# OpenVVC/VVCSoftware_VTM

Hardware: AMD Instinct MI355X
Metric: encoded frames/sec (bit-exact bitstream) at 4K10 RA QP32, 1/2/4/8 GPU [M1: hot-path pictures/s of the kernels behind the call sites, NOT EncoderApp fps] (higher is better)
Workload: dtype int16

## Files before the change

vvcsoftware_vtm_amd/csrc/interp.hip:

```cpp
#include "common.h"
#include "dist_dev.h"
#include "mfma_tr.h"

static_assert(offsetof(vvcgpu_mc_desc, dst_stride) == 32 && offsetof(vvcgpu_mc_desc, w) == 36 && offsetof(vvcgpu_mc_desc, frac_x0) == 40 &&
              offsetof(vvcgpu_mc_desc, is_luma) == 44 && sizeof(vvcgpu_mc_desc) == 48, "vvcgpu_mc_desc layout");

namespace {

__constant__ short c_lumaFilter[16][8] = {
  {  0, 0,   0, 64,  0,   0,  0,  0 }, {  0, 1,  -3, 63,  4,  -2,  1,  0 }, { -1, 2,  -5, 62,  8,  -3,  1,  0 },
  { -1, 3,  -8, 60, 13,  -4,  1,  0 }, { -1, 4, -10, 58, 17,  -5,  1,  0 }, { -1, 4, -11, 52, 26,  -8,  3, -1 },
  { -1, 3,  -9, 47, 31, -10,  4, -1 }, { -1, 4, -11, 45, 34, -10,  4, -1 }, { -1, 4, -11, 40, 40, -11,  4, -1 },
  { -1, 4, -10, 34, 45, -11,  4, -1 }, { -1, 4, -10, 31, 47,  -9,  3, -1 }, { -1, 3,  -8, 26, 52, -11,  4, -1 },
  {  0, 1,  -5, 17, 58, -10,  4, -1 }, {  0, 1,  -4, 13, 60,  -8,  3, -1 }, {  0, 1,  -3,  8, 62,  -5,  2, -1 },
  {  0, 1,  -2,  4, 63,  -3,  1,  0 } };
__constant__ short c_chromaFilter[32][4] = {
  {  0, 64,  0,  0 }, { -1, 63,  2,  0 }, { -2, 62,  4,  0 }, { -2, 60,  7, -1 }, { -2, 58, 10, -2 }, { -3, 57, 12, -2 },
  { -4, 56, 14, -2 }, { -4, 55, 15, -2 }, { -4, 54, 16, -2 }, { -5, 53, 18, -2 }, { -6, 52, 20, -2 }, { -6, 49, 24, -3 },
  { -6, 46, 28, -4 }, { -5, 44, 29, -4 }, { -4, 42, 30, -4 }, { -4, 39, 33, -4 }, { -4, 36, 36, -4 }, { -4, 33, 39, -4 },
  { -4, 30, 42, -4 }, { -4, 29, 44, -5 }, { -4, 28, 46, -6 }, { -3, 24, 49, -6 }, { -2, 20, 52, -6 }, { -2, 18, 53, -5 },
  { -2, 16, 54, -4 }, { -2, 15, 55, -4 }, { -2, 14, 56, -4 }, { -2, 12, 57, -3 }, { -2, 10, 58, -2 }, { -1,  7, 60, -2 },
  {  0,  4, 62, -2 }, {  0,  2, 63, -1 } };

constexpr int IF_INTERNAL_PREC = 14, IF_FILTER_PREC = 6, IF_INTERNAL_OFFS = 1 << 13;
// ... 697 lines not shown
  {
    const int ix = (int)(short)(raw.flg >> 16);
    const vvcgpu_wp_param eA = wp_load(wp, __builtin_amdgcn_readlane(ix, 0)), eB = wp_load(wp, __builtin_amdgcn_readlane(ix, 8));
    o = mm_tail_wp(K, fr[0], fr[1], bi == 1, K.c16 >= 8 ? eB : eA);
  }
  else o = mm_tail(K, fr[0], fr[1], bi == 1 ? 1.f : 0.f, bi == 1 ? K.scBi2 : 1.f, bi == 1 ? K.ofBi2 : 1024.f, bi == 0 && (fx0 | fy0) == 0);
  const bool outB = K.c16 >= 8;
  if ((K.g >> 1) == (K.c16 >> 3) && (outB ? (hasB && !badB) : !badA))
  {
    const long long dstOff = (long long)(((unsigned long long)raw.dstHi << 32) | raw.dstLo);
    Pel* dp = dstBase + dstOff + (ptrdiff_t)(K.c16 & 7) * (int)raw.ds + 4 * (K.g & 1);
    reinterpret_cast<MmQuad*>(dp)->v = o;
  }
}

__device__ __forceinline__ int mm_kind_of(const uint4& q)
{
  vvcgpu_mc_desc d;
  d.w = (short)(q.y & 0xFFFFu); d.h = (short)(q.y >> 16);
  d.frac_x0 = (signed char)(q.z & 0xFFu); d.frac_y0 = (signed char)((q.z >> 8) & 0xFFu); d.frac_x1 = (signed char)((q.z >> 16) & 0xFFu); d.frac_y1 = (signed char)(q.z >> 24);
  d.is_luma = (signed char)(q.w & 0xFFu); d.bi = (signed char)((q.w >> 8) & 0xFFu);
  return mm_kind(d);
}
struct MmServe { const Pel* ref0Base; const Pel* ref1Base; Pel* dstBase; const vvcgpu_mc_desc* descs; const int* flags; int n, bd, cmin, cmax, w0, W, luma; };
struct MmServeWp : MmServe { const vvcgpu_wp_param* wp; int nWp, allGen; };
template <bool WPF> __device__ __forceinline__ void mm_second_pass(const MmServe* sv, short* gen, unsigned* genT);
__device__ __noinline__ void mm_serve_one(const MmServe* sv, int li, short* gen, unsigned* genT);
__device__ __noinline__ void mm_serve_one_wp(const MmServeWp* sv, int li, short* gen, unsigned* genT);
constexpr int MM_SKIP = 3;
__device__ __forceinline__ int mm_wp_kind(int k, const uint4& q2, const vvcgpu_wp_param* __restrict__ wp, int nWp, int bd, int allGen)
{
  if (wp_skip(q2, wp, nWp, bd)) return MM_SKIP;
  return allGen && k > 0 ? 0 : k;
}
constexpr int MM_GEN_SHORTS = 23 * 24 + 23 * 16;

template <int KIND_T>
__global__ __launch_bounds__(256, 4) void mc_mfma_kernel(const Pel* __restrict__ ref0Base, const Pel* __restrict__ ref1Base, Pel* __restrict__ dstBase,
                                                                         const vvcgpu_mc_desc* __restrict__ descs, int n, int bd, int cmin, int cmax,
                                                                         const _Float16* __restrict__ image, int* __restrict__ flags, unsigned long long* __restrict__ diag,
                                                                         int* __restrict__ genCount, int* __restrict__ nextCounters, int serve)
{
  constexpr bool WPF = false;
  const vvcgpu_wp_param* const wp = nullptr;
  const int nWp = 0, allGen = 0;
#include "mc_mfma_body.inc"
}
// ... 203 lines not shown
  static_assert(MM_GEN_SHORTS == WR * WP + WR * ST, "LDS of the generic body inside mc_mfma_kernel");
  const MmServe S = *sv;
  const vvcgpu_mc_desc d = S.descs[li];
  mc_generic_pu<false, 1>(d, S.ref0Base, S.ref1Base, S.dstBase, S.bd, S.cmin, S.cmax, (int)threadIdx.x & 63, gen, gen + WR * WP, genT, nullptr);
}
__device__ __noinline__ void mm_serve_one_wp(const MmServeWp* sv, int li, short* gen, unsigned* genT)
{
  const MmServeWp S = *sv;
  const vvcgpu_mc_desc d = S.descs[li];
  const vvcgpu_wp_param e = wp_load(S.wp, d.reserved);
  mc_generic_pu<false, 2, true>(d, S.ref0Base, S.ref1Base, S.dstBase, S.bd, S.cmin, S.cmax, (int)threadIdx.x & 63, gen, gen + WR * WP, genT, nullptr,
                                &e);
}
template <bool WPF>
__device__ __forceinline__ void mm_second_pass(const MmServe* sv, short* gen, unsigned* genT)
{
  __builtin_amdgcn_fence(__ATOMIC_SEQ_CST, "workgroup");
  const MmServe S = *sv;
  const int lane = (int)threadIdx.x & 63, w = S.w0 + ((int)threadIdx.x >> 6);
  const MmServeWp* svW = static_cast<const MmServeWp*>(sv);
  auto serve = [&](int li) { if constexpr (WPF) mm_serve_one_wp(svW, li, gen, genT); else mm_serve_one(sv, li, gen, genT); };
  if (S.luma)
  {
    for (int j0 = 0; w + (long long)j0 * S.W < S.n; j0 += 64)
    {
      const long long iL = w + (long long)(j0 + lane) * S.W;
      bool gen1 = false;
      if (iL < S.n)
      {
        const uint4 q1 = reinterpret_cast<const uint4*>(S.descs + iL)[1], q2 = reinterpret_cast<const uint4*>(S.descs + iL)[2];
        int k = mm_kind_of(q2);
        const int bi = (int)(signed char)((q2.w >> 8) & 0xFFu);
        if (k == 1 && ((q1.z | (bi == 1 ? q1.w : 0u)) & 7u)) k = -1;
        if constexpr (WPF) k = mm_wp_kind(k, q2, svW->wp, svW->nWp, S.bd, svW->allGen);
        gen1 = k <= 0 || (k == 1 && __hip_atomic_load(S.flags + iL, __ATOMIC_RELAXED, __HIP_MEMORY_SCOPE_AGENT) != 0);
      }
      unsigned long long todo = __ballot(gen1);
      while (todo)
      {
        const int j = (int)__builtin_ctzll(todo);
        todo &= todo - 1ull;
        serve(w + (j0 + j) * S.W);
      }
    }
  }
  else
  {
    const int units = (S.n + 1) >> 1;
    for (int j0 = 0; w + (long long)j0 * S.W < units; j0 += 64)
    {
      const long long uL = w + (long long)(j0 + lane) * S.W;
      int g0 = -1, g1 = -1;
      if (uL < units)
      {
        const uint4* q0 = reinterpret_cast<const uint4*>(S.descs + 2 * uL) + 2;
        const int k0 = WPF ? mm_wp_kind(mm_kind_of(*q0), *q0, svW->wp, svW->nWp, S.bd, svW->allGen) : mm_kind_of(reinterpret_cast<const uint4*>(S.descs + 2 * uL)[2]);
        const int k1 = 2 * uL + 1 < S.n ? (WPF ? mm_wp_kind(mm_kind_of(q0[3]), q0[3], svW->wp, svW->nWp, S.bd, svW->allGen)
                                                : mm_kind_of(reinterpret_cast<const uint4*>(S.descs + 2 * uL + 1)[2])) : 0;
        if (k0 == 2 && __hip_atomic_load(S.flags + 2 * uL, __ATOMIC_RELAXED, __HIP_MEMORY_SCOPE_AGENT) != 0) g0 = (int)(2 * uL);
        if (k1 == 2 && __hip_atomic_load(S.flags + 2 * uL + 1, __ATOMIC_RELAXED, __HIP_MEMORY_SCOPE_AGENT) != 0) g1 = (int)(2 * uL + 1);
      }
      unsigned long long todo = __ballot(g0 >= 0 || g1 >= 0);
      while (todo)
      {
        const int j = (int)__builtin_ctzll(todo);
        todo &= todo - 1ull;
        const int a0 = __builtin_amdgcn_readlane(g0, j), a1 = __builtin_amdgcn_readlane(g1, j);
        if (a0 >= 0) serve(a0);
        if (a1 >= 0) serve(a1);
      }
    }
  }
}

template <bool DIST, bool SUB44 = false>
__global__ __launch_bounds__(64) void mc_batch_kernel(const Pel* __restrict__ ref0Base, const Pel* __restrict__ ref1Base,
// ... 364 lines not shown
```

vvcsoftware_vtm_amd/csrc/mc_mfma_body.inc:

```
  if (blockIdx.x == 0 && threadIdx.x < VVC_CTR_INTS) nextCounters[threadIdx.x] = 0;
  const int KIND = KIND_T ? KIND_T : 1 + ((int)blockIdx.x & 1);
  const int T0 = KIND == 1 ? MM_TAL : MM_TAC, T1 = KIND == 1 ? MM_TAC : MM_ENTRIES;
  __shared__ __align__(16) _Float16 tabL[(KIND_T == 2 ? MM_ENTRIES - MM_TAC : MM_TAC - MM_TAL) * 8];
  __shared__ __align__(16) short genS[4][MM_GEN_SHORTS];
  __shared__ __align__(16) unsigned genT[4][MC_LDS_DW];
  __shared__ typename std::conditional<WPF, MmServeWp, MmServe>::type serveS;
  __shared__ int anyGenS[4];
  for (int i = threadIdx.x; i < T1 - T0; i += 256) reinterpret_cast<uint4*>(tabL)[i] = reinterpret_cast<const uint4*>(image)[T0 + i];
  if (threadIdx.x < 4) anyGenS[threadIdx.x] = 0;
  MmK K;
  K.genCount = serve ? &anyGenS[threadIdx.x >> 6] : genCount;
  K.tabS = tabL - T0 * 8;
  K.lane = threadIdx.x & 63; K.c16 = K.lane & 15; K.g = K.lane >> 4;
  const int g = K.g;
  const int hr = max(2, IF_INTERNAL_PREC - bd), S = 1 << (IF_FILTER_PREC - hr);
  K.hr = hr;
  if constexpr (WPF) { K.cmin = cmin; K.cmax = cmax; }
  K.rangeMask = (unsigned)((1 << bd) - 1) * 0x10001u;
  K.uLo = (unsigned)(16384 + cmin) * 0x10001u; K.uHi = (unsigned)(16384 + cmax) * 0x10001u;
  K.m7[0] = 0x007F007Fu; K.m8[0] = 0x00FF00FFu; K.orX[0] = 0x64006400u;
  asm("" : "+v"(K.m7[0]), "+v"(K.m8[0]), "+v"(K.orX[0]));
  K.orR[0] = K.orX[0];
  K.m7[1] = g < 2 ? 0x007F007Fu : 0u; K.m8[1] = g < 2 ? 0x00FF00FFu : 0u; K.orX[1] = g < 2 ? 0x64006400u : g == 2 ? 0x64003C00u : 0u; K.orR[1] = g < 2 ? 0x64006400u : 0u;
  K.m7[2] = g < 3 ? 0x007F007Fu : 0u; K.m8[2] = g < 3 ? 0x00FF00FFu : 0u; K.orX[2] = g < 3 ? 0x64006400u : 0x64003C00u; K.orR[2] = g < 3 ? 0x64006400u : 0u;
  K.magicN = 8388608.f * (float)S; K.magicH = 536870912.f;
  K.cinN = 8192.f * (float)S - 65536.f - 0.5f * (float)(S - 1); K.cinH = 983040.5f;
  K.perm = (4 * K.c16 + K.g) * 4;
  K.pmin = mm_h2{ (_Float16)(short)(1024 + cmin), (_Float16)(short)(1024 + cmin) }; K.pmax = mm_h2{ (_Float16)(short)(1024 + cmax), (_Float16)(short)(1024 + cmax) };
  K.pmin0 = mm_h2{ (_Float16)1024.f, (_Float16)1024.f }; K.pmaxF = mm_h2{ (_Float16)(short)(1023 + (1 << bd)), (_Float16)(short)(1023 + (1 << bd)) };
  K.scBi1 = 1.f / 64.f; K.scUni1 = 1.f / (float)(64 << hr); K.ofUni1 = (float)((1 << (5 + hr)) + (IF_INTERNAL_OFFS << 6)) * K.scUni1;
  K.scBi2 = 1.f / (float)(2 << hr); K.ofBi2 = (float)((1 << hr) + 2 * IF_INTERNAL_OFFS) * K.scBi2 + 1024.f;

  const int nb = KIND_T ? (int)gridDim.x : (KIND == 1 ? ((int)gridDim.x + 1) >> 1 : (int)gridDim.x >> 1), bi_ = KIND_T ? (int)blockIdx.x : (int)blockIdx.x >> 1;
  const int W = nb * 4, perX = W >> 3;
  const int w = (nb & 7) ? bi_ * 4 + __builtin_amdgcn_readfirstlane((int)threadIdx.x >> 6)
                         : (bi_ & 7) * perX + (bi_ >> 3) * 4 + __builtin_amdgcn_readfirstlane((int)threadIdx.x >> 6);
  if (serve && threadIdx.x == 0) static_cast<MmServe&>(serveS) = MmServe{ ref0Base, ref1Base, dstBase, descs, flags, n, bd, cmin, cmax, w, W, KIND == 1 ? 1 : 0 };
  if constexpr (WPF) { if (threadIdx.x == 0) { MmServeWp& sw = reinterpret_cast<MmServeWp&>(serveS); sw.wp = wp; sw.nWp = nWp; sw.allGen = allGen; } }
  __syncthreads();
  MmRaw raw;
  bool pend = false;
  if (KIND == 1)
  {
    vvcgpu_mc_desc dP = descs[0];
    vvcgpu_wp_param eP;
    int iP = 0, dstep = 0;
    for (int j0 = 0; w + (long long)j0 * W < n; j0 += 64)
    {
      const long long iL = w + (long long)(j0 + K.lane) * W;
      int k = 0;
      if (iL < n)
      {
        const uint4 q1 = reinterpret_cast<const uint4*>(descs + iL)[1], q2 = reinterpret_cast<const uint4*>(descs + iL)[2];
        k = mm_kind_of(q2);
        const int bi = (int)(signed char)((q2.w >> 8) & 0xFFu);
        if (k == 1 && ((q1.z | (bi == 1 ? q1.w : 0u)) & 7u)) k = -1;
        if constexpr (WPF) k = mm_wp_kind(k, q2, wp, nWp, bd, allGen);
        if (k < 0) flags[iL] = 1;
      }
      {
        const unsigned long long gm = __ballot(iL < n && k <= 0);
        if (gm != 0ull && K.lane == 0) atomicAdd(K.genCount, (int)__popcll(gm));
      }
      unsigned long long mine = __ballot(k == 1);
      auto nextIdx = [&]() -> int { if (mine == 0ull) return -1; const int j = (int)__builtin_ctzll(mine); mine &= mine - 1ull; return w + (j0 + j) * W; };
      auto descLoad = [&](int i, uint4 (&v)[3]) { const uint4* q = reinterpret_cast<const uint4*>(descs + i); v[0] = q[0]; v[1] = q[1]; v[2] = q[2]; };
      auto descScalar = [&](const uint4 (&v)[3]) -> vvcgpu_mc_desc
      {
        unsigned u[12] = { v[0].x, v[0].y, v[0].z, v[0].w, v[1].x, v[1].y, v[1].z, v[1].w, v[2].x, v[2].y, v[2].z, v[2].w };
#pragma unroll
        for (int t = 0; t < 12; t++) u[t] = (unsigned)__builtin_amdgcn_readfirstlane((int)u[t]);
        vvcgpu_mc_desc d;
        d.ref0_off = (long long)(((unsigned long long)u[1] << 32) | u[0]); d.ref1_off = (long long)(((unsigned long long)u[3] << 32) | u[2]);
        d.dst_off = (long long)(((unsigned long long)u[5] << 32) | u[4]);
        d.ref0_stride = (int)u[6]; d.ref1_stride = (int)u[7]; d.dst_stride = (int)u[8];
        d.w = (short)(u[9] & 0xFFFFu); d.h = (short)(u[9] >> 16);
        d.frac_x0 = (signed char)(u[10] & 0xFFu); d.frac_y0 = (signed char)((u[10] >> 8) & 0xFFu); d.frac_x1 = (signed char)((u[10] >> 16) & 0xFFu); d.frac_y1 = (signed char)(u[10] >> 24);
        d.is_luma = (signed char)(u[11] & 0xFFu); d.bi = (signed char)((u[11] >> 8) & 0xFFu); d.reserved = WPF ? (short)(u[11] >> 16) : 0;
        return d;
      };
      int iA = nextIdx();
      if (iA < 0) continue;
      uint4 dv[3];
      descLoad(iA, dv);
      while (iA >= 0)
      {
        const vvcgpu_mc_desc dA = descScalar(dv);
        vvcgpu_wp_param eA;
// ... 6 lines not shown
          if (st && K.lane == 0) diag[dstep * 4 + 0] = __builtin_amdgcn_s_memtime();
          MmWin Wn;
          mm_luma_win(K, raw, Wn);
          if (st && K.lane == 0) { asm volatile("" :: "v"(Wn.w[0][0]), "v"(Wn.w[1][1])); diag[dstep * 4 + 1] = __builtin_amdgcn_s_memtime(); }
          mm_fetch_luma(K, dA, ref0Base, ref1Base, raw);
          if (st && K.lane == 0) diag[dstep * 4 + 2] = __builtin_amdgcn_s_memtime();
          mm_luma<WPF>(K, dP, Wn, ref0Base, ref1Base, dstBase, flags, iP, &eP);
          if (st && K.lane == 0) diag[dstep * 4 + 3] = __builtin_amdgcn_s_memtime();
          dstep++;
        }
        else mm_fetch_luma(K, dA, ref0Base, ref1Base, raw);
        dP = dA; iP = iA; pend = true;
        if constexpr (WPF) eP = eA;
        iA = iB;
      }
    }
    if (pend) { MmWin Wn; mm_luma_win(K, raw, Wn); mm_luma<WPF>(K, dP, Wn, ref0Base, ref1Base, dstBase, flags, iP, &eP); }
    if (serve && anyGenS[(int)threadIdx.x >> 6] != 0) mm_second_pass<WPF>(&serveS, genS[(int)threadIdx.x >> 6], genT[(int)threadIdx.x >> 6]);
  }
  else
  {
    const int units = (n + 1) >> 1;
    int iAP = -1, iBP = -1;
    for (int j0 = 0; w + (long long)j0 * W < units; j0 += 64)
    {
      const long long uL = w + (long long)(j0 + K.lane) * W;
      int iAv = -1, iBv = -1;
      if (uL < units)
      {
        const uint4* q0 = reinterpret_cast<const uint4*>(descs + 2 * uL) + 2;
        const int k0 = WPF ? mm_wp_kind(mm_kind_of(*q0), *q0, wp, nWp, bd, allGen) : mm_kind_of(reinterpret_cast<const uint4*>(descs + 2 * uL)[2]);
        const int k1 = 2 * uL + 1 < n ? (WPF ? mm_wp_kind(mm_kind_of(q0[3]), q0[3], wp, nWp, bd, allGen) : mm_kind_of(reinterpret_cast<const uint4*>(descs + 2 * uL + 1)[2])) : 0;
        iAv = k0 == 2 ? (int)(2 * uL) : k1 == 2 ? (int)(2 * uL + 1) : -1;
        iBv = (k0 == 2 && k1 == 2) ? (int)(2 * uL + 1) : -1;
      }
      unsigned long long mine = __ballot(iAv >= 0);
      auto nextJ = [&]() -> int { if (mine == 0ull) return -1; const int j = (int)__builtin_ctzll(mine); mine &= mine - 1ull; return j; };
      int jA = nextJ();
      if (jA < 0) continue;
      int iA = __builtin_amdgcn_readlane(iAv, jA), iB = __builtin_amdgcn_readlane(iBv, jA);
      MmCDesc cA;
      mm_chroma_desc(K, descs, iA, iB, cA);
      while (jA >= 0)
      {
        const int jN = nextJ();
        const int iAN = __builtin_amdgcn_readlane(iAv, jN >= 0 ? jN : jA), iBN = __builtin_amdgcn_readlane(iBv, jN >= 0 ? jN : jA);
        MmCDesc cN;
        mm_chroma_desc(K, descs, iAN, iBN, cN);
        if (pend)
        {
          MmWin Wn;
// ... 13 lines not shown
```

vvcsoftware_vtm_amd/csrc/mehier.hip:

```cpp
#include "common.h"
#include "raster_dev.h"

namespace {

constexpr int MH_PITCH = 148;
constexpr int MH_MAXN = 39;
constexpr int MH_MAXSLOTS = 448;
constexpr int MH_MAXSLIDE = 7;
constexpr int MH_MAXDL = 96;
constexpr unsigned MH_INVALID = 0x30000000u;

struct MhGeom
{
  int n16x, n16y;
  int nsbx, total;
  int refX0, refY0;
  int subShift, hs;
  int nR, R;
  int nD, D;
  int winBytes;
  int dlCount; short dlKey[12]; signed char dlX[48];
  unsigned magicNq, magicDl;
};

// ... 172 lines not shown
  __builtin_amdgcn_s_setprio(0);
  if (nsub == 4)
  {
    mh_block_min(L.kind == 1 ? mh_fold32(a32, L, sh) : 0xFFFFFFFFu, L.idx, &keys[16 + q], lane);
    if (waveHasDense) mh_block_min64(L.kind == 2 ? mh_fold64(a32, L, sh) : ~0ull, &keys[21 + 16 + q], lane);
    if (nsubx == 4 && nsuby == 4)
    {
      unsigned* dst = L.kind == 2 ? surfD + (s - nslots) * 4 : surf + (L.kind ? s : 0) * 4;
      if (L.kind)
      {
#pragma unroll
        for (int m = 0; m < 4; m++) atomicAdd(&dst[m], a32[m]);
      }
      int ticket = 0;
      __builtin_amdgcn_fence(__ATOMIC_RELEASE, "workgroup");
      if (lane == 0) ticket = atomicAdd(arrive, 1);
      __builtin_amdgcn_fence(__ATOMIC_ACQUIRE, "workgroup");
      ticket = __builtin_amdgcn_readfirstlane(ticket);
      if (ticket == 3)
      {
        unsigned a[4];
#pragma unroll
        for (int m = 0; m < 4; m++) a[m] = L.kind ? dst[m] : 0u;
        mh_block_min(L.kind == 1 ? mh_fold32(a, L, sh) : 0xFFFFFFFFu, L.idx, &keys[20], lane);
        if (waveHasDense) mh_block_min64(L.kind == 2 ? mh_fold64(a, L, sh) : ~0ull, &keys[41], lane);
      }
    }
  }
}

__global__ __launch_bounds__(1024) void me_hier_kernel(const unsigned* orgPacked, const Pel* __restrict__ ref, int rs, MhGeom g, vvcgpu_mvcost mv,
                                                       vvcgpu_search_best* __restrict__ r16, vvcgpu_search_best* __restrict__ r32, vvcgpu_search_best* __restrict__ r64,
                                                       vvcgpu_search_best* __restrict__ d16, vvcgpu_search_best* __restrict__ d32, vvcgpu_search_best* __restrict__ d64,
                                                       unsigned long long* __restrict__ diagArg)
{
#ifdef MH_DIAG
  unsigned long long* const diag = diagArg;
#endif
  extern __shared__ __align__(16) unsigned refL[];
  __shared__ unsigned long long keys[42];
  __shared__ unsigned costTab[R5C_COST_N];
  __shared__ unsigned char bitsRX[MH_MAXN + 1], bitsRY[MH_MAXN + 1], bitsDX[12], bitsDY[12];
  __shared__ short dlKey[12];
  __shared__ signed char dlX[12 * 4];
  __shared__ unsigned surfD[MH_MAXDL * 4];
  __shared__ int arrive[8];
  __shared__ vvcgpu_search_best* outPtr[6];
  __shared__ vvcgpu_mvcost mvL;
  const int tid = threadIdx.x, lane = tid & 63;
  const int chunk = (g.total + 7) >> 3;
  for (int n = tid; n < R5C_COST_N; n += (int)blockDim.x) costTab[n] = (unsigned)(unsigned long long)(mv.lambda * (double)n);
  if (tid == 700) { outPtr[0] = r16; outPtr[1] = r32; outPtr[2] = r64; outPtr[3] = d16; outPtr[4] = d32; outPtr[5] = d64; mvL = mv; }
  if (tid >= 512 && tid < 512 + 12) dlKey[tid - 512] = g.dlKey[tid - 512];
  if (tid >= 576 && tid < 576 + 48) dlX[tid - 576] = g.dlX[tid - 576];
  if (tid < 2 * g.nR)
  {
    const int n = tid < g.nR ? tid : tid - g.nR;
    const int v = tid < g.nR ? (((-g.R + 5 * n) << mv.cost_scale) - mv.pred_hor) : (((-g.R + 5 * n) << mv.cost_scale) - mv.pred_ver);
    (tid < g.nR ? bitsRX : bitsRY)[n] = (unsigned char)expgolomb_bits(v >> mv.imv_shift);
  }
  else if (tid >= 128 && tid < 128 + 2 * g.nD)
  {
    const int t = tid - 128, n = t < g.nD ? t : t - g.nD;
    const int v = t < g.nD ? (((-g.D + n) << mv.cost_scale) - mv.pred_hor) : (((-g.D + n) << mv.cost_scale) - mv.pred_ver);
    (t < g.nD ? bitsDX : bitsDY)[n] = (unsigned char)expgolomb_bits(v >> mv.imv_shift);
  }
  __syncthreads();
  const int wave = __builtin_amdgcn_readfirstlane(tid >> 6), nwaves = (int)(blockDim.x >> 6);
  const unsigned ldsBase = (unsigned)(size_t)(__attribute__((address_space(3))) unsigned*)refL;
  const int off = (int)(((ptrdiff_t)(g.refY0 - g.R) * rs + g.refX0 - g.R) & 7);
  const int nq = (g.nR + 3) >> 2, nslots = g.nR * nq, ndl = g.nD * g.dlCount, nsw = (nslots + ndl + 63) >> 6;
  MhLane LU[2];
  {
    MhTables T = { costTab, bitsRX, bitsRY, bitsDX, bitsDY, dlKey, dlX, g.dlCount };
#pragma unroll
    for (int r = 0; r < 2; r++)
    {
      const int u = wave + r * nwaves, sw = nsw - 1 - (u >> 2);
      LU[r].kind = 0; LU[r].base = 0; LU[r].idx = 0; LU[r].cst[0] = LU[r].cst[1] = LU[r].cst[2] = LU[r].cst[3] = MH_INVALID << 2;
      if (u < 4 * nsw) mh_lane(sw * 64 + lane, g, T, off, nq, nslots, ndl, LU[r]);
    }
  }
  const int perX = (int)(gridDim.x >> 3), runLen = (chunk + perX - 1) / perX, kk0 = (int)(blockIdx.x >> 3) * runLen;
  int slide = 0, pfQ0 = 0;
  bool pfHave = false;
  uint4 pf[2];
  int sbyRun = ((int)(blockIdx.x & 7) * chunk + kk0) / g.nsbx, sbxRun = ((int)(blockIdx.x & 7) * chunk + kk0) - sbyRun * g.nsbx;
  for (int kk = kk0; kk < kk0 + runLen && kk < chunk; kk++)
  {
  const int item = (int)(blockIdx.x & 7) * chunk + kk;
  if (item >= g.total) break;
  const int sby = sbyRun, sbx = sbxRun;
  if (++sbxRun == g.nsbx) { sbxRun = 0; sbyRun++; }
  const int nsubx = min(4, g.n16x - 4 * sbx), nsuby = min(4, g.n16y - 4 * sby);
#ifdef MH_DIAG
  const bool stamp = diag && item == (g.total >> 1) + 3;
  const int stampK = item == (g.total >> 2) ? 0 : item == (g.total >> 3) ? 1 : item == 3 * (g.total >> 2) ? 2 : item == 5 * (g.total >> 3) ? 3 : -1;
#else
  constexpr bool stamp = false;
  constexpr int stampK = -1;
  unsigned long long* const diag = nullptr;
#endif
  if (diag && stampK >= 0 && tid == 0) diag[40 + 0 * 4 + stampK] = __builtin_amdgcn_s_memtime();
  if (stamp && tid == 0) diag[0] = __builtin_amdgcn_s_memtime();
  unsigned* surf = refL + (g.winBytes >> 2);

  const int winCols = (g.nR - 1) * 5 + 16 * nsubx, winRows = (g.nR - 1) * 5 + 16 * nsuby - (1 << g.subShift) + 1;
  const ptrdiff_t winOff = (ptrdiff_t)(g.refY0 + 64 * sby - g.R) * rs + g.refX0 + 64 * sbx - g.R;
  const int nQuads = ((winCols - 1 + off) >> 3) + 1;
  const int rsQ = rs >> 3;
  auto slideItem = [&](int it, int q0, int& row, int& q) { row = it >> 3; q = q0 + (it & 7); };
  if (pfHave)
  {
    slide++;
    unsigned* winL = refL + slide * 32;
#pragma unroll
    for (int u = 0; u < 2; u++)
    {
      const int it = tid + u * 1024;
      if (it < 8 * winRows)
      {
        int row, q;
        slideItem(it, pfQ0, row, q);
        uint2* d = reinterpret_cast<uint2*>(winL + row * MH_PITCH + 4 * q);
        d[0] = make_uint2(pf[u].x ^ 0x80008000u, pf[u].y ^ 0x80008000u);
        d[1] = make_uint2(pf[u].z ^ 0x80008000u, pf[u].w ^ 0x80008000u);
      }
    }
  }
  else
  {
    slide = 0;
    fill_window_cols<9>(refL, reinterpret_cast<const uint4*>(ref + (winOff - off)), rs >> 3, winRows, MH_PITCH, nQuads, tid, (int)blockDim.x);
  }
  pfHave = false;
  if (kk + 1 < kk0 + runLen && kk + 1 < chunk && item + 1 < g.total && sbx + 1 < g.nsbx && slide < MH_MAXSLIDE)
  {
    const int nsubxN = min(4, g.n16x - 4 * (sbx + 1)), nQuadsN = (((g.nR - 1) * 5 + 16 * nsubxN - 1 + off) >> 3) + 1;
    pfQ0 = nQuads - 8;
    if (nQuadsN - pfQ0 == 8 && 8 * winRows <= 2048)
    {
      pfHave = true;
      const uint4* gsrc = reinterpret_cast<const uint4*>(ref + (winOff + 64 - off));
#pragma unroll
      for (int u = 0; u < 2; u++)
      {
        const int it = tid + u * 1024;
        pf[u] = make_uint4(0u, 0u, 0u, 0u);
        if (it < 8 * winRows)
        {
          int row, q;
          slideItem(it, pfQ0, row, q);
          pf[u] = gsrc[(size_t)row * rsQ + q];
        }
      }
    }
  }
  if (tid < 42) keys[tid] = ~0ull;
  if (tid >= 64 && tid < 72) arrive[tid - 64] = 0;
  if (tid < MH_MAXDL * 4) surfD[tid] = 0u;
  for (int n = tid; n < MH_MAXSLOTS * 4; n += (int)blockDim.x) surf[n] = 0u;
  asm volatile("s_waitcnt lgkmcnt(0)\n\ts_barrier" ::: "memory");
  if (stamp && tid == 0) diag[1] = __builtin_amdgcn_s_memtime();
  if (diag && stampK >= 0 && tid == 0) diag[40 + 1 * 4 + stampK] = __builtin_amdgcn_s_memtime();

#pragma unroll 1
  for (int r = 0; r < 2; r++)
  {
    const int u = wave + r * nwaves;
    if (u < 4 * nsw)
    {
      const int sw = nsw - 1 - (u >> 2), q = u & 3;
      const int s = sw * 64 + lane;
      const bool waveHasDense = ndl > 0 && sw * 64 + 63 >= nslots;
      MhLane L;
      L.base = r ? LU[1].base : LU[0].base; L.idx = r ? LU[1].idx : LU[0].idx; L.kind = r ? LU[1].kind : LU[0].kind;
#pragma unroll
      for (int m = 0; m < 4; m++) L.cst[m] = r ? LU[1].cst[m] : LU[0].cst[m];
      mh_unit(orgPacked, g, off & 3, ldsBase + (unsigned)(slide * 128 + (q & 1) * 64 + (q >> 1) * 32 * MH_PITCH * 4), L, waveHasDense, q, sbx, sby, nsubx, nsuby, keys, surf, surfD, &arrive[sw], s, nslots, lane);
      if (stamp && lane == 0) diag[8 + u] = __builtin_amdgcn_s_memtime();
    }
  }
  __syncthreads();
  if (stamp && tid == 0) diag[2] = diag[3] = __builtin_amdgcn_s_memtime();
  if (diag && stampK >= 0 && tid == 0) diag[40 + 2 * 4 + stampK] = __builtin_amdgcn_s_memtime();

  if (tid < 42)
  {
    const int grid = tid >= 21, t = tid - 21 * grid;
    vvcgpu_search_best* out = nullptr; int bidx = 0; bool exists = false;
    if (t < 16)      { const int tx = t & 3, ty = t >> 2; exists = tx < nsubx && ty < nsuby; bidx = (4 * sby + ty) * g.n16x + 4 * sbx + tx; out = outPtr[grid * 3]; }
    else if (t < 20) { const int qx = (t - 16) & 1, qy = (t - 16) >> 1; exists = 2 * qx + 2 <= nsubx && 2 * qy + 2 <= nsuby; bidx = (2 * sby + qy) * (g.n16x >> 1) + 2 * sbx + qx; out = outPtr[grid * 3 + 1]; }
    else             { exists = nsubx == 4 && nsuby == 4; bidx = sby * (g.n16x >> 2) + sbx; out = outPtr[grid * 3 + 2]; }
    if (exists && out && !(grid && !g.nD))
    {
      const unsigned long long key = keys[tid];
      const int idx = (int)(key & 0xFFFFFFu);
      const unsigned long long cost = key >> 24;
      const int n = grid ? g.nD : g.nR, step = grid ? 1 : 5, p0 = grid ? -g.D : -g.R;
      const int j = (int)(((float)idx + 0.5f) * __frcp_rn((float)n)), i = idx - j * n;
      const int x = p0 + i * step, y = p0 + j * step;
      const unsigned bits = grid ? (unsigned)bitsDX[i] + bitsDY[j] : (unsigned)bitsRX[i] + bitsRY[j];
      vvcgpu_search_best r;
      r.x = x; r.y = y; r.cost = cost; r.sad = cost - (unsigned long long)costTab[bits];
      out[bidx] = r;
    }
  }
  }
}

}

extern "C" {

int vvcgpu_me_hier_search(const vvc_pel* org, int org_stride, const vvc_pel* ref, int ref_stride, const vvcgpu_me_hier_cfg* cfg_host,
                          const vvcgpu_mvcost* mvcost_host, vvcgpu_search_best* const* raster_best, vvcgpu_search_best* const* dense_best, void* stream)
{
  VVC_CHECK_ARG(org && ref && cfg_host && mvcost_host && raster_best, "me_hier_search: null pointer");
  const vvcgpu_me_hier_cfg c = *cfg_host;
  VVC_CHECK_ARG(c.n16x >= 1 && c.n16y >= 1 && c.n16x <= 4096 && c.n16y <= 4096, "me_hier_search: grid %d x %d", c.n16x, c.n16y);
  VVC_CHECK_ARG(c.raster_step == 5 && c.raster_range >= 5 && c.dense_range >= 0, "me_hier_search: raster step %d range %d, dense range %d", c.raster_step, c.raster_range, c.dense_range);
  VVC_CHECK_ARG(raster_best[0] && (c.n16x < 2 || c.n16y < 2 || raster_best[1]) && (c.n16x < 4 || c.n16y < 4 || raster_best[2]), "me_hier_search: raster result arrays");
  VVC_CHECK_ARG(c.dense_range == 0 || (dense_best && dense_best[0] && (c.n16x < 2 || c.n16y < 2 || dense_best[1]) && (c.n16x < 4 || c.n16y < 4 || dense_best[2])),
                "me_hier_search: dense result arrays");
  const int nR = 2 * (c.raster_range / 5) + 1, R = 5 * (c.raster_range / 5), nD = c.dense_range ? 2 * c.dense_range + 1 : 0;
  if (nR > MH_MAXN || nD > 9 || (c.dense_range && R < c.dense_range + 15) || c.sub_shift < 0 || c.sub_shift > 1 || (org_stride & 1) || (ref_stride & 7) || ((uintptr_t)org & 3) || ((uintptr_t)ref & 15) ||
      !(mvcost_host->lambda >= 0.0 && mvcost_host->lambda < 4.0e6))
  {
    vvcgpu_set_error("me_hier_search: shape outside the hierarchical kernel (raster +-%d, +-%d grid, sub_shift %d, strides %d / %d, lambda %g)",
                     c.raster_range, c.dense_range, c.sub_shift, org_stride, ref_stride, mvcost_host->lambda);
    return VVCGPU_E_UNSUPPORTED;
// ... 4 lines not shown
  g.refX0 = c.ref_x; g.refY0 = c.ref_y; g.subShift = c.sub_shift; g.hs = 16 >> c.sub_shift;
  g.nR = nR; g.R = R; g.nD = nD; g.D = c.dense_range;
  g.dlCount = 0;
  g.magicNq = (65536u + (unsigned)((nR + 3) >> 2) - 1u) / (unsigned)((nR + 3) >> 2);
  memset(g.dlKey, 0, sizeof g.dlKey); memset(g.dlX, -128, sizeof g.dlX);
  for (int x = -c.dense_range; x <= c.dense_range && nD; x++)
  {
    const int m = (R + x) & 3, key = (R + x - 5 * m) >> 2;
    int l = 0;
    while (l < g.dlCount && g.dlKey[l] != key) l++;
    if (l == g.dlCount) g.dlKey[g.dlCount++] = (short)key;
    g.dlX[4 * l + m] = (signed char)x;
  }
  g.magicDl = g.dlCount ? (65536u + (unsigned)g.dlCount - 1u) / (unsigned)g.dlCount : 0u;
  const int winRowsMax = (nR - 1) * 5 + 64;
  g.winBytes = winRowsMax * MH_PITCH * 4 + MH_MAXSLIDE * 128 + 128;
  const size_t smem = (size_t)g.winBytes + MH_MAXSLOTS * 4 * sizeof(unsigned);
  const int nblocks = c.n16x * c.n16y;
  VvcScratch sc(st);
  unsigned* packed = sc.take<unsigned>((size_t)nblocks * g.hs * 16);
  if (!packed) return VVCGPU_E_DEVICE;
  hipLaunchKernelGGL(mh_pack_org_kernel, dim3((unsigned)(((size_t)nblocks * g.hs * 4 + 255) / 256)), dim3(256), 0, st, org, org_stride, c.org_x, c.org_y, c.n16x, nblocks, g.hs, c.sub_shift, packed);
  VVC_LAUNCH_CHECK();
  VVC_HIP(hipFuncSetAttribute(reinterpret_cast<const void*>(me_hier_kernel), hipFuncAttributeMaxDynamicSharedMemorySize, (int)smem));
  unsigned long long* diag = nullptr;
#ifdef MH_DIAG
  const bool wantDiag = getenv("VVCGPU_MH_DIAG") != nullptr;
#else
  const bool wantDiag = false;
#endif
  if (wantDiag) { VVC_HIP(hipMalloc(&diag, 64 * sizeof(unsigned long long))); VVC_HIP(hipMemsetAsync(diag, 0, 64 * sizeof(unsigned long long), st)); }
  const char* wgsEnv = getenv("VVCGPU_MH_WGS");
  const int wgsMax = wgsEnv && atoi(wgsEnv) >= 8 ? (atoi(wgsEnv) / 8) * 8 : (vvcgpu_cu_count() / 8) * 8;
  const int gridWgs = min(cdiv(g.total, 8) * 8, wgsMax);
  hipLaunchKernelGGL(me_hier_kernel, dim3(gridWgs), dim3(1024), smem, st, packed, ref, ref_stride, g, *mvcost_host,
                     raster_best[0], raster_best[1], raster_best[2], dense_best ? dense_best[0] : nullptr, dense_best ? dense_best[1] : nullptr, dense_best ? dense_best[2] : nullptr, diag);
  VVC_LAUNCH_CHECK();
  if (wantDiag)
  {
    unsigned long long h[64];
    VVC_HIP(hipStreamSynchronize(st));
    VVC_HIP(hipMemcpy(h, diag, sizeof h, hipMemcpyDeviceToHost));
    (void)hipFree(diag);
    fprintf(stderr, "[vvcgpu me_hier diag] cycles: window staged %llu, units done %llu, 64x64 pass %llu; per unit end (since start):", h[1] - h[0], h[2] - h[0], h[3] - h[0]);
    for (int u = 0; u < 32; u++) if (h[8 + u]) fprintf(stderr, " %llu", h[8 + u] - h[0]);
    fprintf(stderr, "\n[vvcgpu me_hier diag] four more workgroups (window staged / all done):");
    for (int k = 0; k < 4; k++) fprintf(stderr, " %llu / %llu", h[44 + k] - h[40 + k], h[48 + k] - h[40 + k]);
    fprintf(stderr, "\n");
  }
  return VVCGPU_OK;
}

}
```

Before: 2007.

## Chunk MC descriptor walk and overlap ME record writes with next super-block

The MC MFMA kernel walks descriptors in contiguous chunks when n is large and the grid is a multiple of 16, so the walk has better locality across workgroups. It recovers the PU index with a readlane instead of recomputing it. The hierarchical ME kernel double-buffers the key and geometry arrays. Each super-block's result records are written by the last wave while the next super-block is processed, and per-item reset work moves into the units or to kernel start. The host sets the max dynamic shared memory attribute once per device using a worst-case size instead of on every call. The changes add indexing complexity, and correctness depends on resetting keys, arrive and surf inside the units.

```diff
diff --git a/vvcsoftware_vtm_amd/csrc/interp.hip b/vvcsoftware_vtm_amd/csrc/interp.hip
--- a/vvcsoftware_vtm_amd/csrc/interp.hip
+++ b/vvcsoftware_vtm_amd/csrc/interp.hip
@@ -743,7 +743,28 @@
   d.is_luma = (signed char)(q.w & 0xFFu); d.bi = (signed char)((q.w >> 8) & 0xFFu);
   return mm_kind(d);
 }
-struct MmServe { const Pel* ref0Base; const Pel* ref1Base; Pel* dstBase; const vvcgpu_mc_desc* descs; const int* flags; int n, bd, cmin, cmax, w0, W, luma; };
+struct MmServe { const Pel* ref0Base; const Pel* ref1Base; Pel* dstBase; const vvcgpu_mc_desc* descs; const int* flags; int n, bd, cmin, cmax, w0, W, luma, c0, nch; };
+constexpr int MM_CHUNK_MIN_N = 8192;
+__device__ __forceinline__ int mm_walk_chunks(int n, int nblocks)
+{
+  if (n < MM_CHUNK_MIN_N || (nblocks & 15)) return 0;
+  const int m = (int)(((long long)n + 12288) / 24576);
+  return 8 * (m < 1 ? 1 : m);
+}
+struct MmWalk { int w, W, c0, nch, csz, spc, N, T; };
+__device__ __forceinline__ MmWalk mm_walk_of(int N, int w, int W, int c0, int nch)
+{
+  MmWalk k = { w, W, c0, nch, (N + nch - 1) / nch, 0, N, 0 };
+  k.spc = (k.csz + W - 1) / W;
+  k.T = c0 < nch ? ((nch - c0 + 7) >> 3) * k.spc : 0;
+  return k;
+}
+__device__ __forceinline__ int mm_walk_index(const MmWalk& k, int t)
+{
+  const int ci = (int)((unsigned)t / (unsigned)k.spc), j = t - ci * k.spc, c = k.c0 + 8 * ci;
+  const long long i = (long long)c * k.csz + k.w + (long long)j * k.W, ce = (long long)(c + 1) * k.csz;
+  return c < k.nch && i < ce && i < k.N ? (int)i : -1;
+}
 struct MmServeWp : MmServe { const vvcgpu_wp_param* wp; int nWp, allGen; };
 template <bool WPF> __device__ __forceinline__ void mm_second_pass(const MmServe* sv, short* gen, unsigned* genT);
 __device__ __noinline__ void mm_serve_one(const MmServe* sv, int li, short* gen, unsigned* genT);
@@ -993,11 +1014,12 @@
   auto serve = [&](int li) { if constexpr (WPF) mm_serve_one_wp(svW, li, gen, genT); else mm_serve_one(sv, li, gen, genT); };
   if (S.luma)
   {
-    for (int j0 = 0; w + (long long)j0 * S.W < S.n; j0 += 64)
-    {
-      const long long iL = w + (long long)(j0 + lane) * S.W;
+    const MmWalk wk = mm_walk_of(S.n, w, S.W, S.c0, S.nch);
+    for (int j0 = 0; j0 < wk.T; j0 += 64)
+    {
+      const int iL = mm_walk_index(wk, j0 + lane);
       bool gen1 = false;
-      if (iL < S.n)
+      if (iL >= 0)
       {
         const uint4 q1 = reinterpret_cast<const uint4*>(S.descs + iL)[1], q2 = reinterpret_cast<const uint4*>(S.descs + iL)[2];
         int k = mm_kind_of(q2);
@@ -1011,18 +1033,19 @@
       {
         const int j = (int)__builtin_ctzll(todo);
         todo &= todo - 1ull;
-        serve(w + (j0 + j) * S.W);
+        serve(__builtin_amdgcn_readlane(iL, j));
       }
     }
   }
   else
   {
     const int units = (S.n + 1) >> 1;
-    for (int j0 = 0; w + (long long)j0 * S.W < units; j0 += 64)
-    {
-      const long long uL = w + (long long)(j0 + lane) * S.W;
+    const MmWalk wk = mm_walk_of(units, w, S.W, S.c0, S.nch);
+    for (int j0 = 0; j0 < wk.T; j0 += 64)
+    {
+      const long long uL = mm_walk_index(wk, j0 + lane);
       int g0 = -1, g1 = -1;
-      if (uL < units)
+      if (uL >= 0)
       {
         const uint4* q0 = reinterpret_cast<const uint4*>(S.descs + 2 * uL) + 2;
         const int k0 = WPF ? mm_wp_kind(mm_kind_of(*q0), *q0, svW->wp, svW->nWp, S.bd, svW->allGen) : mm_kind_of(reinterpret_cast<const uint4*>(S.descs + 2 * uL)[2]);
diff --git a/vvcsoftware_vtm_amd/csrc/mc_mfma_body.inc b/vvcsoftware_vtm_amd/csrc/mc_mfma_body.inc
--- a/vvcsoftware_vtm_amd/csrc/mc_mfma_body.inc
+++ b/vvcsoftware_vtm_amd/csrc/mc_mfma_body.inc
@@ -1,5 +1,6 @@
   if (blockIdx.x == 0 && threadIdx.x < VVC_CTR_INTS) nextCounters[threadIdx.x] = 0;
-  const int KIND = KIND_T ? KIND_T : 1 + ((int)blockIdx.x & 1);
+  const int nch = KIND_T ? 0 : mm_walk_chunks(n, (int)gridDim.x);
+  const int KIND = KIND_T ? KIND_T : 1 + (nch ? ((int)blockIdx.x >> 3) & 1 : (int)blockIdx.x & 1);
   const int T0 = KIND == 1 ? MM_TAL : MM_TAC, T1 = KIND == 1 ? MM_TAC : MM_ENTRIES;
   __shared__ __align__(16) _Float16 tabL[(KIND_T == 2 ? MM_ENTRIES - MM_TAC : MM_TAC - MM_TAL) * 8];
   __shared__ __align__(16) short genS[4][MM_GEN_SHORTS];
@@ -31,11 +32,12 @@
   K.scBi1 = 1.f / 64.f; K.scUni1 = 1.f / (float)(64 << hr); K.ofUni1 = (float)((1 << (5 + hr)) + (IF_INTERNAL_OFFS << 6)) * K.scUni1;
   K.scBi2 = 1.f / (float)(2 << hr); K.ofBi2 = (float)((1 << hr) + 2 * IF_INTERNAL_OFFS) * K.scBi2 + 1024.f;
 
-  const int nb = KIND_T ? (int)gridDim.x : (KIND == 1 ? ((int)gridDim.x + 1) >> 1 : (int)gridDim.x >> 1), bi_ = KIND_T ? (int)blockIdx.x : (int)blockIdx.x >> 1;
-  const int W = nb * 4, perX = W >> 3;
-  const int w = (nb & 7) ? bi_ * 4 + __builtin_amdgcn_readfirstlane((int)threadIdx.x >> 6)
-                         : (bi_ & 7) * perX + (bi_ >> 3) * 4 + __builtin_amdgcn_readfirstlane((int)threadIdx.x >> 6);
-  if (serve && threadIdx.x == 0) static_cast<MmServe&>(serveS) = MmServe{ ref0Base, ref1Base, dstBase, descs, flags, n, bd, cmin, cmax, w, W, KIND == 1 ? 1 : 0 };
+  const int nb = KIND_T ? (int)gridDim.x : (KIND == 1 ? ((int)gridDim.x + 1) >> 1 : (int)gridDim.x >> 1), bi_ = KIND_T ? (int)blockIdx.x : nch ? (((int)blockIdx.x >> 4) << 3) | ((int)blockIdx.x & 7) : (int)blockIdx.x >> 1;
+  const int wave_ = __builtin_amdgcn_readfirstlane((int)threadIdx.x >> 6);
+  const int W = nch ? ((int)gridDim.x >> 4) * 4 : nb * 4, perX = W >> 3;
+  const int w = nch ? ((int)blockIdx.x >> 4) * 4 + wave_ : (nb & 7) ? bi_ * 4 + wave_ : (bi_ & 7) * perX + (bi_ >> 3) * 4 + wave_;
+  const int c0 = nch ? (int)blockIdx.x & 7 : 0, nchW = nch ? nch : 1;
+  if (serve && threadIdx.x == 0) static_cast<MmServe&>(serveS) = MmServe{ ref0Base, ref1Base, dstBase, descs, flags, n, bd, cmin, cmax, w, W, KIND == 1 ? 1 : 0, c0, nchW };
   if constexpr (WPF) { if (threadIdx.x == 0) { MmServeWp& sw = reinterpret_cast<MmServeWp&>(serveS); sw.wp = wp; sw.nWp = nWp; sw.allGen = allGen; } }
   __syncthreads();
   MmRaw raw;
@@ -45,11 +47,12 @@
     vvcgpu_mc_desc dP = descs[0];
     vvcgpu_wp_param eP;
     int iP = 0, dstep = 0;
-    for (int j0 = 0; w + (long long)j0 * W < n; j0 += 64)
+    const MmWalk wk = mm_walk_of(n, w, W, c0, nchW);
+    for (int j0 = 0; j0 < wk.T; j0 += 64)
     {
-      const long long iL = w + (long long)(j0 + K.lane) * W;
+      const int iL = mm_walk_index(wk, j0 + K.lane);
       int k = 0;
-      if (iL < n)
+      if (iL >= 0)
       {
         const uint4 q1 = reinterpret_cast<const uint4*>(descs + iL)[1], q2 = reinterpret_cast<const uint4*>(descs + iL)[2];
         k = mm_kind_of(q2);
@@ -59,11 +62,11 @@
         if (k < 0) flags[iL] = 1;
       }
       {
-        const unsigned long long gm = __ballot(iL < n && k <= 0);
+        const unsigned long long gm = __ballot(iL >= 0 && k <= 0);
         if (gm != 0ull && K.lane == 0) atomicAdd(K.genCount, (int)__popcll(gm));
       }
       unsigned long long mine = __ballot(k == 1);
-      auto nextIdx = [&]() -> int { if (mine == 0ull) return -1; const int j = (int)__builtin_ctzll(mine); mine &= mine - 1ull; return w + (j0 + j) * W; };
+      auto nextIdx = [&]() -> int { if (mine == 0ull) return -1; const int j = (int)__builtin_ctzll(mine); mine &= mine - 1ull; return __builtin_amdgcn_readlane(iL, j); };
       auto descLoad = [&](int i, uint4 (&v)[3]) { const uint4* q = reinterpret_cast<const uint4*>(descs + i); v[0] = q[0]; v[1] = q[1]; v[2] = q[2]; };
       auto descScalar = [&](const uint4 (&v)[3]) -> vvcgpu_mc_desc
       {
@@ -116,11 +119,12 @@
   {
     const int units = (n + 1) >> 1;
     int iAP = -1, iBP = -1;
-    for (int j0 = 0; w + (long long)j0 * W < units; j0 += 64)
+    const MmWalk wk = mm_walk_of(units, w, W, c0, nchW);
+    for (int j0 = 0; j0 < wk.T; j0 += 64)
     {
-      const long long uL = w + (long long)(j0 + K.lane) * W;
+      const long long uL = mm_walk_index(wk, j0 + K.lane);
       int iAv = -1, iBv = -1;
-      if (uL < units)
+      if (uL >= 0)
       {
         const uint4* q0 = reinterpret_cast<const uint4*>(descs + 2 * uL) + 2;
         const int k0 = WPF ? mm_wp_kind(mm_kind_of(*q0), *q0, wp, nWp, bd, allGen) : mm_kind_of(reinterpret_cast<const uint4*>(descs + 2 * uL)[2]);
diff --git a/vvcsoftware_vtm_amd/csrc/mehier.hip b/vvcsoftware_vtm_amd/csrc/mehier.hip
--- a/vvcsoftware_vtm_amd/csrc/mehier.hip
+++ b/vvcsoftware_vtm_amd/csrc/mehier.hip
@@ -1,5 +1,6 @@
 #include "common.h"
 #include "raster_dev.h"
+#include <atomic>
 
 namespace {
 
@@ -218,9 +219,43 @@
         unsigned a[4];
 #pragma unroll
         for (int m = 0; m < 4; m++) a[m] = L.kind ? dst[m] : 0u;
+        if (L.kind)
+        {
+#pragma unroll
+          for (int m = 0; m < 4; m++) dst[m] = 0u;
+        }
+        if (lane == 0) *arrive = 0;
         mh_block_min(L.kind == 1 ? mh_fold32(a, L, sh) : 0xFFFFFFFFu, L.idx, &keys[20], lane);
         if (waveHasDense) mh_block_min64(L.kind == 2 ? mh_fold64(a, L, sh) : ~0ull, &keys[41], lane);
       }
+    }
+  }
+}
+
+struct MhRecTabs { const unsigned* costTab; const unsigned char* bitsRX; const unsigned char* bitsRY; const unsigned char* bitsDX; const unsigned char* bitsDY; };
+__device__ __forceinline__ void mh_write_records(int lane, unsigned long long* keysB, const int* geo, const MhGeom& g, vvcgpu_search_best* const* outPtr, const MhRecTabs& T)
+{
+  if (lane < 42)
+  {
+    const int sbx = geo[0], sby = geo[1], nsubx = geo[2], nsuby = geo[3];
+    const int grid = lane >= 21, t = lane - 21 * grid;
+    const unsigned long long key = keysB[lane];
+    keysB[lane] = ~0ull;
+    vvcgpu_search_best* out = nullptr; int bidx = 0; bool exists = false;
+    if (t < 16)      { const int tx = t & 3, ty = t >> 2; exists = tx < nsubx && ty < nsuby; bidx = (4 * sby + ty) * g.n16x + 4 * sbx + tx; out = outPtr[grid * 3]; }
+    else if (t < 20) { const int qx = (t - 16) & 1, qy = (t - 16) >> 1; exists = 2 * qx + 2 <= nsubx && 2 * qy + 2 <= nsuby; bidx = (2 * sby + qy) * (g.n16x >> 1) + 2 * sbx + qx; out = outPtr[grid * 3 + 1]; }
+    else             { exists = nsubx == 4 && nsuby == 4; bidx = sby * (g.n16x >> 2) + sbx; out = outPtr[grid * 3 + 2]; }
+    if (exists && out && !(grid && !g.nD))
+    {
+      const int idx = (int)(key & 0xFFFFFFu);
+      const unsigned long long cost = key >> 24;
+      const int n = grid ? g.nD : g.nR, step = grid ? 1 : 5, p0 = grid ? -g.D : -g.R;
+      const int j = (int)(((float)idx + 0.5f) * __frcp_rn((float)n)), i = idx - j * n;
+      const int x = p0 + i * step, y = p0 + j * step;
+      const unsigned bits = grid ? (unsigned)T.bitsDX[i] + T.bitsDY[j] : (unsigned)T.bitsRX[i] + T.bitsRY[j];
+      vvcgpu_search_best r;
+      r.x = x; r.y = y; r.cost = cost; r.sad = cost - (unsigned long long)T.costTab[bits];
+      out[bidx] = r;
     }
   }
 }
@@ -234,7 +269,8 @@
   unsigned long long* const diag = diagArg;
 #endif
   extern __shared__ __align__(16) unsigned refL[];
-  __shared__ unsigned long long keys[42];
+  __shared__ unsigned long long keys[2][42];
+  __shared__ int geoL[2][4];
   __shared__ unsigned costTab[R5C_COST_N];
   __shared__ unsigned char bitsRX[MH_MAXN + 1], bitsRY[MH_MAXN + 1], bitsDX[12], bitsDY[12];
   __shared__ short dlKey[12];
@@ -261,6 +297,11 @@
     const int v = t < g.nD ? (((-g.D + n) << mv.cost_scale) - mv.pred_hor) : (((-g.D + n) << mv.cost_scale) - mv.pred_ver);
     (t < g.nD ? bitsDX : bitsDY)[n] = (unsigned char)expgolomb_bits(v >> mv.imv_shift);
   }
+  unsigned* const surf = refL + (g.winBytes >> 2);
+  if (tid < 84) (&keys[0][0])[tid] = ~0ull;
+  if (tid >= 64 && tid < 72) arrive[tid - 64] = 0;
+  if (tid < MH_MAXDL * 4) surfD[tid] = 0u;
+  for (int n = tid; n < MH_MAXSLOTS * 4; n += (int)blockDim.x) surf[n] = 0u;
   __syncthreads();
   const int wave = __builtin_amdgcn_readfirstlane(tid >> 6), nwaves = (int)(blockDim.x >> 6);
   const unsigned ldsBase = (unsigned)(size_t)(__attribute__((address_space(3))) unsigned*)refL;
@@ -282,25 +323,28 @@
   bool pfHave = false;
   uint4 pf[2];
   int sbyRun = ((int)(blockIdx.x & 7) * chunk + kk0) / g.nsbx, sbxRun = ((int)(blockIdx.x & 7) * chunk + kk0) - sbyRun * g.nsbx;
-  for (int kk = kk0; kk < kk0 + runLen && kk < chunk; kk++)
+  const MhRecTabs RT = { costTab, bitsRX, bitsRY, bitsDX, bitsDY };
+  const int kkEnd = min(min(kk0 + runLen, chunk), g.total - (int)(blockIdx.x & 7) * chunk);
+  for (int kk = kk0; kk < kkEnd; kk++)
   {
   const int item = (int)(blockIdx.x & 7) * chunk + kk;
-  if (item >= g.total) break;
+  const int kb = (kk - kk0) & 1;
   const int sby = sbyRun, sbx = sbxRun;
   if (++sbxRun == g.nsbx) { sbxRun = 0; sbyRun++; }
   const int nsubx = min(4, g.n16x - 4 * sbx), nsuby = min(4, g.n16y - 4 * sby);
 #ifdef MH_DIAG
   const bool stamp = diag && item == (g.total >> 1) + 3;
+  const bool stampPrev = diag && item == (g.total >> 1) + 4;
+  const bool stampF = diag && item == (g.total >> 1);
   const int stampK = item == (g.total >> 2) ? 0 : item == (g.total >> 3) ? 1 : item == 3 * (g.total >> 2) ? 2 : item == 5 * (g.total >> 3) ? 3 : -1;
 #else
-  constexpr bool stamp = false;
+  constexpr bool stamp = false, stampPrev = false, stampF = false;
   constexpr int stampK = -1;
   unsigned long long* const diag = nullptr;
 #endif
   if (diag && stampK >= 0 && tid == 0) diag[40 + 0 * 4 + stampK] = __builtin_amdgcn_s_memtime();
   if (stamp && tid == 0) diag[0] = __builtin_amdgcn_s_memtime();
-  unsigned* surf = refL + (g.winBytes >> 2);
-
+  if (stampF && tid == 0) diag[52] = __builtin_amdgcn_s_memtime();
   const int winCols = (g.nR - 1) * 5 + 16 * nsubx, winRows = (g.nR - 1) * 5 + 16 * nsuby - (1 << g.subShift) + 1;
   const ptrdiff_t winOff = (ptrdiff_t)(g.refY0 + 64 * sby - g.R) * rs + g.refX0 + 64 * sbx - g.R;
   const int nQuads = ((winCols - 1 + off) >> 3) + 1;
@@ -330,7 +374,7 @@
     fill_window_cols<9>(refL, reinterpret_cast<const uint4*>(ref + (winOff - off)), rs >> 3, winRows, MH_PITCH, nQuads, tid, (int)blockDim.x);
   }
   pfHave = false;
-  if (kk + 1 < kk0 + runLen && kk + 1 < chunk && item + 1 < g.total && sbx + 1 < g.nsbx && slide < MH_MAXSLIDE)
+  if (kk + 1 < kkEnd && sbx + 1 < g.nsbx && slide < MH_MAXSLIDE)
   {
     const int nsubxN = min(4, g.n16x - 4 * (sbx + 1)), nQuadsN = (((g.nR - 1) * 5 + 16 * nsubxN - 1 + off) >> 3) + 1;
     pfQ0 = nQuads - 8;
@@ -352,12 +396,10 @@
       }
     }
   }
-  if (tid < 42) keys[tid] = ~0ull;
-  if (tid >= 64 && tid < 72) arrive[tid - 64] = 0;
-  if (tid < MH_MAXDL * 4) surfD[tid] = 0u;
-  for (int n = tid; n < MH_MAXSLOTS * 4; n += (int)blockDim.x) surf[n] = 0u;
+  if (tid == 64) { geoL[kb][0] = sbx; geoL[kb][1] = sby; geoL[kb][2] = nsubx; geoL[kb][3] = nsuby; }
   asm volatile("s_waitcnt lgkmcnt(0)\n\ts_barrier" ::: "memory");
   if (stamp && tid == 0) diag[1] = __builtin_amdgcn_s_memtime();
+  if (stampF && tid == 0) diag[53] = __builtin_amdgcn_s_memtime();
   if (diag && stampK >= 0 && tid == 0) diag[40 + 1 * 4 + stampK] = __builtin_amdgcn_s_memtime();
 
 #pragma unroll 1
@@ -373,36 +415,25 @@
       L.base = r ? LU[1].base : LU[0].base; L.idx = r ? LU[1].idx : LU[0].idx; L.kind = r ? LU[1].kind : LU[0].kind;
 #pragma unroll
       for (int m = 0; m < 4; m++) L.cst[m] = r ? LU[1].cst[m] : LU[0].cst[m];
-      mh_unit(orgPacked, g, off & 3, ldsBase + (unsigned)(slide * 128 + (q & 1) * 64 + (q >> 1) * 32 * MH_PITCH * 4), L, waveHasDense, q, sbx, sby, nsubx, nsuby, keys, surf, surfD, &arrive[sw], s, nslots, lane);
+      mh_unit(orgPacked, g, off & 3, ldsBase + (unsigned)(slide * 128 + (q & 1) * 64 + (q >> 1) * 32 * MH_PITCH * 4), L, waveHasDense, q, sbx, sby, nsubx, nsuby, keys[kb], surf, surfD, &arrive[sw], s, nslots, lane);
       if (stamp && lane == 0) diag[8 + u] = __builtin_amdgcn_s_memtime();
     }
+  }
+  if (wave == nwaves - 1 && kk > kk0)
+  {
+    if (stampPrev && lane == 0) diag[5] = __builtin_amdgcn_s_memtime();
+    __builtin_amdgcn_s_setprio(3);
+    mh_write_records(lane, keys[kb ^ 1], geoL[kb ^ 1], g, outPtr, RT);
+    __builtin_amdgcn_s_setprio(0);
+    if (stampPrev && lane == 0) diag[6] = __builtin_amdgcn_s_memtime();
   }
   __syncthreads();
   if (stamp && tid == 0) diag[2] = diag[3] = __builtin_amdgcn_s_memtime();
+  if (stampF && tid == 0) diag[54] = diag[55] = __builtin_amdgcn_s_memtime();
+  if (stamp && tid == 0) diag[4] = __builtin_amdgcn_s_memtime();
   if (diag && stampK >= 0 && tid == 0) diag[40 + 2 * 4 + stampK] = __builtin_amdgcn_s_memtime();
-
-  if (tid < 42)
-  {
-    const int grid = tid >= 21, t = tid - 21 * grid;
-    vvcgpu_search_best* out = nullptr; int bidx = 0; bool exists = false;
-    if (t < 16)      { const int tx = t & 3, ty = t >> 2; exists = tx < nsubx && ty < nsuby; bidx = (4 * sby + ty) * g.n16x + 4 * sbx + tx; out = outPtr[grid * 3]; }
-    else if (t < 20) { const int qx = (t - 16) & 1, qy = (t - 16) >> 1; exists = 2 * qx + 2 <= nsubx && 2 * qy + 2 <= nsuby; bidx = (2 * sby + qy) * (g.n16x >> 1) + 2 * sbx + qx; out = outPtr[grid * 3 + 1]; }
-    else             { exists = nsubx == 4 && nsuby == 4; bidx = sby * (g.n16x >> 2) + sbx; out = outPtr[grid * 3 + 2]; }
-    if (exists && out && !(grid && !g.nD))
-    {
-      const unsigned long long key = keys[tid];
-      const int idx = (int)(key & 0xFFFFFFu);
-      const unsigned long long cost = key >> 24;
-      const int n = grid ? g.nD : g.nR, step = grid ? 1 : 5, p0 = grid ? -g.D : -g.R;
-      const int j = (int)(((float)idx + 0.5f) * __frcp_rn((float)n)), i = idx - j * n;
-      const int x = p0 + i * step, y = p0 + j * step;
-      const unsigned bits = grid ? (unsigned)bitsDX[i] + bitsDY[j] : (unsigned)bitsRX[i] + bitsRY[j];
-      vvcgpu_search_best r;
-      r.x = x; r.y = y; r.cost = cost; r.sad = cost - (unsigned long long)costTab[bits];
-      out[bidx] = r;
-    }
-  }
-  }
+  }
+  if (wave == nwaves - 1 && kkEnd > kk0) mh_write_records(lane, keys[(kkEnd - 1 - kk0) & 1], geoL[(kkEnd - 1 - kk0) & 1], g, outPtr, RT);
 }
 
 }
@@ -453,7 +484,17 @@
   if (!packed) return VVCGPU_E_DEVICE;
   hipLaunchKernelGGL(mh_pack_org_kernel, dim3((unsigned)(((size_t)nblocks * g.hs * 4 + 255) / 256)), dim3(256), 0, st, org, org_stride, c.org_x, c.org_y, c.n16x, nblocks, g.hs, c.sub_shift, packed);
   VVC_LAUNCH_CHECK();
-  VVC_HIP(hipFuncSetAttribute(reinterpret_cast<const void*>(me_hier_kernel), hipFuncAttributeMaxDynamicSharedMemorySize, (int)smem));
+  {
+    static std::atomic<int> attrSet[64];
+    int dev = 0;
+    VVC_HIP(hipGetDevice(&dev));
+    if (dev < 0 || dev >= 64 || !attrSet[dev].load(std::memory_order_acquire))
+    {
+      const int smemMax = ((MH_MAXN - 1) * 5 + 64) * MH_PITCH * 4 + MH_MAXSLIDE * 128 + 128 + MH_MAXSLOTS * 4 * (int)sizeof(unsigned);
+      VVC_HIP(hipFuncSetAttribute(reinterpret_cast<const void*>(me_hier_kernel), hipFuncAttributeMaxDynamicSharedMemorySize, smemMax));
+      if (dev >= 0 && dev < 64) attrSet[dev].store(1, std::memory_order_release);
+    }
+  }
   unsigned long long* diag = nullptr;
 #ifdef MH_DIAG
   const bool wantDiag = getenv("VVCGPU_MH_DIAG") != nullptr;
@@ -475,6 +516,13 @@
     (void)hipFree(diag);
     fprintf(stderr, "[vvcgpu me_hier diag] cycles: window staged %llu, units done %llu, 64x64 pass %llu; per unit end (since start):", h[1] - h[0], h[2] - h[0], h[3] - h[0]);
     for (int u = 0; u < 32; u++) if (h[8 + u]) fprintf(stderr, " %llu", h[8 + u] - h[0]);
+    {
+      unsigned long long lo = ~0ull, hi = 0ull;
+      for (int wv = 0; wv < 16; wv++) { const unsigned long long e = h[8 + 16 + wv] ? h[8 + 16 + wv] : h[8 + wv]; if (e) { lo = e < lo ? e : lo; hi = e > hi ? e : hi; } }
+      fprintf(stderr, "\n[vvcgpu me_hier diag] slide super-block: T_win %llu, T_units %llu, first / last wave done %llu / %llu (spread %llu), loop body ends %llu (T_rec %llu); record writers %llu",
+              h[1] - h[0], h[2] - h[1], lo - h[0], hi - h[0], hi - lo, h[4] - h[0], h[4] - h[2], h[6] - h[5]);
+      fprintf(stderr, "\n[vvcgpu me_hier diag] refill super-block: T_win %llu, T_units %llu, T_rec %llu", h[53] - h[52], h[54] - h[53], h[55] - h[54]);
+    }
     fprintf(stderr, "\n[vvcgpu me_hier diag] four more workgroups (window staged / all done):");
     for (int k = 0; k < 4; k++) fprintf(stderr, " %llu / %llu", h[44 + k] - h[40 + k], h[48 + k] - h[40 + k]);
     fprintf(stderr, "\n");
```

Result: no change. 2030 (median of 4 runs) (+1.1%).
